# sxontheway/milliEye

Hardware: AMD Instinct MI355X
Metric: frames/sec YOLOv3-416+fusion @batch32, 1/2/4/8 MI355X; mAP@0.5 vs ref (higher is better)
Workload: dtype f32; 1 GPU; yolov3.cfg 416x416 fp32 inference, batch=32 per GPU, full milliEye: Darknet.forward -> NMS -> Network.forward mode 0 (R-CNN head + radar fusion, 2 radar boxes/frame) -> output rows, synthetic frames U[0,1), deterministic trained-like weights; stage=full, batch_per_gpu=32, global_batch=32, img_size=416, parallelism=frames sharded over 1 GPU(s), one process per GPU, no data-path collective, rccl_ranks=0, full=False, output_rows_last_step=6449, rois_last_step=6449

## Files before the change

### millieye_amd/csrc/conv.hip

```cpp
#include <stdlib.h>

#include "common.h"
#include "dma.h"

#include "conv32_common.h"

namespace me32 {
int launch_p8_tile(const ConvP& p, int tile, hipStream_t stream);
bool ws1x1_f32_eligible(const ConvP& p);
int launch_ws1x1_f32(const ConvP& p, hipStream_t stream);
bool ws3x3_f32_eligible(const ConvP& p);
int launch_ws3x3_f32(const ConvP& p, hipStream_t stream);
bool stem_mfma_eligible(const ConvP& p);
int launch_stem_mfma(const ConvP& p, hipStream_t stream);
}

namespace {

template <int BM, int BN, int BK, int WR, int WC, int ABL = 0, int PRIO = 0>
__global__ __launch_bounds__(256) void conv_igemm_f32(ConvP p) {
  static_assert(WR * WC == 4, "4 waves per workgroup");
  constexpr int TM = BM / WR, TN = BN / WC;
  constexpr int MT = TM / 32, NT = TN / 32;
  static_assert(MT >= 1 && NT >= 1, "wave tile must hold at least one 32x32 MFMA tile");
  constexpr int LP = BK + 4;
  constexpr int CH = BK / 4;
  constexpr int A_IT = (BM * CH + 255) / 256;
  constexpr int B_IT = (BN * CH + 255) / 256;

  extern __shared__ __attribute__((aligned(16))) float smem[];
  float* As = smem;
  float* Bs = smem + 2 * BM * LP;

  const int tid = threadIdx.x;
  const int lane = tid & 63;
  const int wave = tid >> 6;
  const int wr = wave / WC, wc = wave % WC;
// ... 1303 lines not shown
  p.cs = p.stages = p.tiles_m = p.tiles_n = p.bulk = p.gn = p.kord = 0;
  p.partial = nullptr;
  p.splitk = 1;
  p.sps = 0;
  p.counters = d->tile_counters_len > 0 ? d->tile_counters : nullptr;
  p.counters_len = p.counters ? d->tile_counters_len : 0;
  p.mask_cols = d->tap_mask_cols > 0 ? d->tap_mask_cols : 0;
  for (int i = 0; i < 4; ++i) p.tapmask[i] = d->tap_mask[i];
  return 0;
}

}

extern "C" {

int64_t me_conv2d_flops(const me_conv_desc* d) {
  if (!d) return 0;
  return 2ll * d->n * d->ho * d->wo * (int64_t)d->cout * d->ksize * d->ksize * d->cin;
}

int64_t me_conv2d_workspace_bytes(const me_conv_desc* d) {
  ConvP p;
  if (!d || fill_params(d, p) != 0 || d->cin <= 4) return 0;
  if ((d->tile >= 41 && d->tile <= 45) || d->tile == 47) {
    static const int shape[7][2] = {{128, 128}, {128, 64}, {64, 64}, {128, 32}, {256, 128}, {0, 0}, {64, 64}};
    const int bm = shape[d->tile - 41][0], bn = shape[d->tile - 41][1];
    const long long tiles = (long long)((p.M + bm - 1) / bm) * ((p.cout + bn - 1) / bn);
    const int split = d->split_k > 0 ? d->split_k : 4;
    return (int64_t)(tiles % 256) * split * bm * bn * (int64_t)sizeof(float);
  }
  const ConvPlan plan = plan_conv(p, d->tile, d->split_k > 0 ? d->split_k : kMaxSplit);
  const int split = d->split_k > 0 ? d->split_k : plan.splitk;
  return split > 1 ? (int64_t)split * p.M * p.cout * (int64_t)sizeof(float) : 0;
}

int me_conv2d_f32(const me_conv_desc* d, void* stream_) {
  hipStream_t stream = reinterpret_cast<hipStream_t>(stream_);
  ConvP p;
  int rc = fill_params(d, p);
  if (rc) return rc;
  ME_REQUIRE(d->x && d->wgt && d->scale && d->shift && d->y, ME_E_NULLPTR, "me_conv2d_f32: null tensor pointer");
  ME_REQUIRE(d->upsample == 1 || d->upsample == 2, ME_E_BADARG, "me_conv2d_f32: upsample must be 1 or 2");
  ME_REQUIRE(d->act >= 0 && d->act <= 2, ME_E_BADARG, "me_conv2d_f32: unknown activation %d", d->act);
  ME_REQUIRE(d->y_pitch >= d->cout, ME_E_BADARG, "me_conv2d_f32: y_pitch < cout");

  if (d->cin <= 4) {
    ME_REQUIRE(d->ksize == 3, ME_E_BADARG, "me_conv2d_f32: cin <= 4 needs ksize 3 (direct stem kernel)");
    ME_REQUIRE(d->cout <= SC_MAXCOUT, ME_E_TOOBIG, "me_conv2d_f32: small-cin kernel supports cout <= %d", SC_MAXCOUT);
    ME_REQUIRE(d->res == nullptr && d->upsample == 1, ME_E_BADARG,
               "me_conv2d_f32: small-cin kernel has no residual/upsample epilogue");
    ME_REQUIRE(d->x_nchw || d->x_pitch >= d->cin, ME_E_BADARG, "me_conv2d_f32: x_pitch < cin");
    ME_REQUIRE(me::aligned16(d->y), ME_E_ALIGN, "me_conv2d_f32: y not 16-byte aligned");
    if (d->tile == 0 && me32::stem_mfma_eligible(p)) return me32::launch_stem_mfma(p, stream);
    if (d->cin == 3 && (d->y_pitch & 3) == 0 && d->tile != 91) {
      const unsigned mb = (unsigned)((p.M + 255) / 256);
      if (d->cout % 32 == 0) {
        hipLaunchKernelGGL(conv_stem3_f32<32>, dim3(mb, d->cout / 32), dim3(256), 0, stream, p);
        return me::check_launch("conv_stem3_f32");
      }
      if (d->cout % 16 == 0) {
        hipLaunchKernelGGL(conv_stem3_f32<16>, dim3(mb, d->cout / 16), dim3(256), 0, stream, p);
        return me::check_launch("conv_stem3_f32");
      }
    }
    const long long threads = (long long)p.M * (((p.cout + 7) & ~7) >> 3);
    const unsigned blocks = (unsigned)((threads + 255) / 256);
    if (d->cin == 3)
// ... 101 lines not shown
```

### millieye_amd/engine.py

```python
import ctypes as C
import json
import os
import time

import torch

from . import hip, planner
from .planner import pick_tap_module

__all__ = ["DarknetEngine", "ConvWeights", "pick_tap_module", "invalidate_weights", "bump_versions"]

_EPOCH = [0]


def invalidate_weights():
    _EPOCH[0] += 1


def bump_versions(*tensors):
    torch.autograd.graph.increment_version(tensors)

_DTYPES = ("f32", "bf16", "f16")
_TORCH_HALF = {"bf16": torch.bfloat16, "f16": torch.float16}


class ConvWeights:

    def __init__(self, conv, bn=None, dtype="f32", cin_pad=0, cout_pad=0):
        self.conv, self.bn = conv, bn
        self.dtype, self.cin_pad, self.cout_pad = dtype, cin_pad, cout_pad
        self.wgt = self.scale = self.shift = None
        self.wgt_tiled = None
        self.want_rot = False
        self.rot = self.rot_tiled = None
        self.want_parity, self.parity, self.parity_stamp = False, None, None
        self._stamp = None

    def _sources(self):
        cp = self.conv._parameters
        ts = [cp["weight"]]
        if cp.get("bias") is not None:
            ts.append(cp["bias"])
        if self.bn is not None:
            bp, bb = self.bn._parameters, self.bn._buffers
            ts += [bp["weight"], bp["bias"], bb["running_mean"], bb["running_var"]]
        return ts

    def stamp(self):
        return tuple((t.data_ptr(), t._version) for t in self._sources()) + (_EPOCH[0],)

    def _prepare_packed_f32(self, device):
        conv, bn = self.conv, self.bn
        w = conv.weight
        cout, cin, k, k2 = w.shape
        if k != k2:
            return None
        srcs = [w] + [t for t in ((conv.bias,) if conv.bias is not None else ())]
        if bn is not None:
            srcs += [bn.weight, bn.bias, bn.running_mean, bn.running_var]
        if not all(t.device == device and t.dtype == torch.float32 and t.is_contiguous() for t in srcs):
            return None
        f32 = dict(device=device, dtype=torch.float32)
        realloc = self.wgt is None or self.wgt.device != device or tuple(self.wgt.shape) != (cout, k, k, cin) \
            or self.wgt.dtype != torch.float32
        if realloc:
            self.wgt = torch.empty((cout, k, k, cin), **f32)
            self.scale, self.shift = torch.empty(cout, **f32), torch.empty(cout, **f32)
            self.wgt_tiled = torch.empty((k * k, cin // 16, cout, 16), **f32) if cin % 16 == 0 else None
            self.rot = self.rot_tiled = None
        if self.want_rot and self.rot is None:
            self.rot = torch.empty((cin, k, k, cout), **f32)
            self.rot_tiled = torch.empty((k * k, cout // 16, cin, 16), **f32) if cout % 16 == 0 else None
        if realloc:
            self.parity = None
        if self.want_parity and k == 3 and self.parity is None:
            self.parity = torch.empty((4 * cin, 2, 2, cout), **f32)
        return "realloc" if realloc else True

    def _pack_desc(self, d):
        conv, bn = self.conv, self.bn
        ptr = lambda t: t.data_ptr() if t is not None else None
        cout, cin, k, _ = conv.weight.shape
        d.w, d.bias = conv.weight.data_ptr(), ptr(conv.bias)
        d.gamma, d.beta = ptr(bn.weight if bn is not None else None), ptr(bn.bias if bn is not None else None)
        d.mean, d.var = ptr(bn.running_mean if bn is not None else None), ptr(bn.running_var if bn is not None else None)
        d.ohwi, d.tiled = self.wgt.data_ptr(), ptr(self.wgt_tiled)
        d.rot, d.rot_tiled = ptr(self.rot if self.want_rot else None), ptr(self.rot_tiled if self.want_rot else None)
        d.scale, d.shift = self.scale.data_ptr(), self.shift.data_ptr()
        d.parity = ptr(self.parity if self.want_parity else None)
        d.cout, d.cin, d.ksize, d.eps = cout, cin, k, float(bn.eps) if bn is not None else 0.0
        return d

    def _refresh_packed_f32(self, device):
        done = self._prepare_packed_f32(device)
        if done is None:
            return None
        self.parity_stamp = None
        d = self._pack_desc(hip.PackDesc())
        hip.check(hip.lib().me_pack_conv_f32(d.w, d.cout, d.cin, d.ksize, d.bias, d.gamma, d.beta, d.mean, d.var, d.eps, d.ohwi,
                                             d.tiled, d.rot, d.rot_tiled, d.scale, d.shift, hip.stream_ptr()),
                  "me_pack_conv_f32")
        return done

    def refresh(self, device):
        stamp = self.stamp() + (self.want_rot,)
        if stamp == self._stamp and self.wgt is not None and self.wgt.device == device:
            return False
        dev = torch.device(device)
        if self.dtype == "f32" and not self.cin_pad and not self.cout_pad and dev.type == "cuda":
            if dev.index is None:
                dev = torch.device("cuda", torch.cuda.current_device())
            done = self._refresh_packed_f32(dev)
            if done is not None:
                self._stamp = stamp
                return done
        with torch.no_grad():
            w = self.conv.weight.detach().to(device=device, dtype=torch.float32)
            packed = w.permute(0, 2, 3, 1).contiguous()
            cout = w.shape[0]
            if self.bn is not None:
                g = self.bn.weight.detach().to(device, torch.float64)
                b = self.bn.bias.detach().to(device, torch.float64)
                mean = self.bn.running_mean.detach().to(device, torch.float64)
                var = self.bn.running_var.detach().to(device, torch.float64)
                scale = g / torch.sqrt(var + self.bn.eps)
                shift = b - mean * scale
                if self.conv.bias is not None:
# ... 112 lines not shown
            for cw, _ in stale:
                if cw.refresh(dev) == "realloc" and self._plans:
                    self._plans.clear()
            return
        if "realloc" in states and self._plans:
            self._plans.clear()
        descs = (hip.PackDesc * len(stale))()
        for d, (cw, _) in zip(descs, stale):
            cw._pack_desc(d)
        key = bytes(descs)
        cached = self.__dict__.get("_pack_table")
        if cached is None or cached[0] != key:
            total = int(hip.lib().me_pack_conv_plan(descs, len(stale)))
            if total <= 0:
                raise hip.MeError("me_pack_conv_plan: " + hip.lib().me_last_error().decode("utf-8", "replace"))
            table = torch.frombuffer(bytearray(bytes(descs)), dtype=torch.uint8).to(dev)
            cached = self._pack_table = (key, table, total, max(int(d.ksize) for d in descs))
        _, table, total, max_k = cached
        hip.check(hip.lib().me_pack_conv_batch_f32(table.data_ptr(), len(stale), total, max_k, hip.stream_ptr()),
                  "me_pack_conv_batch_f32")
        for cw, stamp in stale:
            cw._stamp = stamp
            cw.parity_stamp = stamp if cw.parity is not None else None

    def refresh_weights(self, device):
        fast = self.__dict__.get("_fast_sources")
        if fast is None:
            slots, bns = [], []
            for i, d in enumerate(self.model.module_defs):
                if d["type"] != "convolutional":
                    continue
                seq = self.model.module_list[i]
                conv = seq[0]
                slots.append((conv._parameters, "weight"))
                if conv._parameters.get("bias") is not None:
                    slots.append((conv._parameters, "bias"))
                if len(seq) > 1 and isinstance(seq[1], torch.nn.BatchNorm2d):
                    bn = seq[1]
                    bns.append(bn)
                    slots += [(bn._parameters, "weight"), (bn._parameters, "bias"), (bn._buffers, "running_mean"),
                              (bn._buffers, "running_var")]
            fast = self._fast_sources = (slots, bns)
            self._fast_stamp = None
        slots, bns = fast
        for bn in bns:
            if bn.training:
# ... 19 lines not shown
        return tuple([(t.data_ptr(), t._version) for t in [dct[key] for dct, key in fast[0]]]) + (str(device), _EPOCH[0])

    def _build(self, n, h, w, device, keep_raw=False):
        defs, tap = self.model.module_defs, self.tap_module
        half = self.dtype in _TORCH_HALF
        ops, tensors, out, yolo_rows = planner.lower(defs, int(self.model.hyperparams["channels"]), h, w, tap, half, keep_raw,
                                                     decode_last=os.environ.get("MILLIEYE_DECODE_LAST", "1") != "0")
        tap_tensor = out[tap] if tap is not None and tap < len(defs) else None
        total = planner.place(ops, tensors, n, tap_tensor, keep_raw)

        plan = _Plan()
        plan.n, plan.h, plan.w = n, h, w
        plan.arena = torch.empty(max(total, planner._ALIGN), dtype=torch.uint8, device=device)
        if plan.arena.data_ptr() % planner._ALIGN:
            raise RuntimeError("the caching allocator returned an arena that is not 256-byte aligned")
        plan.arena_bytes = total
        plan.dtype = self.dtype
        plan.rows = sum(yolo_rows)
        lib = hip.lib()
        self._emit(plan, ops, device, lib)
        self._attach_workspace(plan, device, lib)
        if _autotune_enabled():
            _autotune(plan, lib)
        plan.fused_blocks = []
        if half and _bneck_mode() != "0" and (_autotune_enabled() or _bneck_mode() == "force"):
            _fuse_bottlenecks(plan, ops, lib)
        if tap_tensor is not None:
            plan.tap = _typed_view(plan, tap_tensor, nchw=True)
            plan.tap_ptr, plan.tap_pitch = _view(plan, tap_tensor)
            plan.tap_shape = (tap_tensor.h, tap_tensor.w, tap_tensor.c)
        else:
            plan.tap = None
        return plan

    def _emit(self, plan, ops, device, lib):
        n, half = plan.n, plan.dtype in _TORCH_HALF
        half_type = hip.HALF_TYPES[_TORCH_HALF[plan.dtype]] if half else 0
        plan.num_classes = None
        plan.input_descs = []
        plan.yolo_raw = []
        plan.yolo_descs = []
        plan.conv_descs = []
        plan.conv_flops = 0
        plan.launches = launches = []
        for op in ops:
            kind, x, y, dsc = op["kind"], op.get("x"), op.get("y"), None
            if kind == "conv":
                op["launch"] = len(launches)
                dsc = op["desc"] = self._conv_desc(plan, op, device, half_type)
                fn = lib.me_conv2d_h16 if half else lib.me_conv2d_f32
            elif kind == "pool" and half:
                fn = lib.me_maxpool_h16
                args = (*_view(plan, x), *_view(plan, y), n, x.h, x.w, x.c, op["k"], op["s"],
                        0 if op["zero_ext"] else op["pad"], op["zero_ext"], op["ho"], op["wo"], half_type)
            elif kind == "pool":
                dsc = hip.PoolDesc()
                dsc.x, dsc.x_pitch = _view(plan, x)
                dsc.y, dsc.y_pitch = _view(plan, y)
                dsc.n, dsc.h, dsc.w, dsc.c = n, x.h, x.w, x.c
                dsc.size, dsc.stride, dsc.pad, dsc.zero_ext = op["k"], op["s"], (0 if op["zero_ext"] else op["pad"]), \
                    op["zero_ext"]
                dsc.ho, dsc.wo = op["ho"], op["wo"]
                fn = lib.me_maxpool_f32
            elif kind == "upsample":
                fn = lib.me_upsample_h16 if x.esize == 2 else lib.me_upsample_f32
# ... 23 lines not shown
            self._plans.clear()
        dsc = hip.Conv16Desc() if half else hip.ConvDesc()
        if x.external:
            dsc.x, dsc.x_pitch, dsc.x_nchw = None, x.c, 1
            plan.input_descs.append(dsc)
        else:
            dsc.x, dsc.x_pitch = _view(plan, x)
            dsc.x_nchw = 0
        dsc.wgt, dsc.scale, dsc.shift = cw.wgt.data_ptr(), cw.scale.data_ptr(), cw.shift.data_ptr()
        if op["res"] is not None:
            dsc.res, dsc.res_pitch = _view(plan, op["res"])
        else:
            dsc.res, dsc.res_pitch = None, 0
        dsc.y, dsc.y_pitch = _view(plan, y)
        dsc.n, dsc.h, dsc.w, dsc.cin = plan.n, x.h, x.w, x.c
        dsc.cout, dsc.ksize, dsc.stride, dsc.pad = cw.wgt.shape[0], op["k"], op["s"], op["pad"]
        dsc.ho, dsc.wo, dsc.act, dsc.upsample, dsc.tile = op["ho"], op["wo"], op["act"], op["ups"], 0
        dsc.split_k, dsc.workspace, dsc.workspace_bytes = 0, None, 0
        dsc.wgt_tiled = cw.wgt_tiled.data_ptr() if cw.wgt_tiled is not None else None
        if half:
            dsc.y_f32 = 1 if y.esize == 4 else 0
            dsc.half_type = half_type
        plan.conv_descs.append((op["module"], dsc))
        plan.conv_flops += 2 * plan.n * op["ho"] * op["wo"] * op["cout"] * op["k"] * op["k"] * (x.c - x.padded)
        return dsc

    def _yolo_desc(self, plan, op):
        x, i = op["x"], op["module"]
        yl = self.model.module_list[i][0]
        na, nc = yl.num_anchors, yl.num_classes
        if x.c != na * (nc + 5):
            raise ValueError(f"yolo {i}: {x.c} channels != {na}*({nc}+5)")
        dsc = hip.YoloDesc()
        dsc.x, dsc.x_pitch = _view(plan, x)
        dsc.out = None
        dsc.n, dsc.g, dsc.num_anchors, dsc.num_classes = plan.n, op["g"], na, nc
        dsc.rows_total, dsc.row_offset = plan.rows, op["row_offset"]
        stride = plan.h / op["g"]
        dsc.stride = stride
        for k, (aw, ah) in enumerate(yl.anchors):
            dsc.anchors[2 * k] = aw / stride
            dsc.anchors[2 * k + 1] = ah / stride
        plan.num_classes = nc
        plan.yolo_descs.append(dsc)
        plan.yolo_raw.append(_typed_view(plan, x, nchw=False))
        yl.img_dim = plan.h
# ... 201 lines not shown
    if _TUNE_FILE_LOADED[0]:
        return
    _TUNE_FILE_LOADED[0] = True
    try:
        with open(_tune_file()) as fh:
            for k, v in json.load(fh).items():
                _TUNE_CACHE[tuple(int(x) for x in k.split(","))] = (int(v[0]), int(v[1]))
    except (OSError, ValueError):
        pass


def _tune_save():
    path = _tune_file()
    try:
        os.makedirs(os.path.dirname(path), exist_ok=True)
        tmp = f"{path}.{os.getpid()}.tmp"
        with open(tmp, "w") as fh:
            json.dump({",".join(str(int(x)) for x in k): list(v) for k, v in _TUNE_CACHE.items()}, fh)
        os.replace(tmp, path)
    except OSError:
        pass


def _autotune(plan, lib):

    stream = hip.stream_ptr()
    _tune_load()
    bf16 = plan.dtype in _TORCH_HALF
    conv_fn = lib.me_conv2d_h16 if bf16 else lib.me_conv2d_f32
    todo, keyed = [], []
    for _m, d in plan.conv_descs:
        if d.cin <= 4:
            continue
        key = (d.n, d.h, d.w, d.cin, d.cout, d.ksize, d.stride, d.upsample, int(bool(d.res)))
        if bf16:
            key += (16 + d.y_f32 + 2 * d.half_type,)
        keyed.append((key, d))
        hit = _TUNE_CACHE.get(key)
        if hit is not None:
            d.tile, d.split_k = hit
        else:
            todo.append((key, d))

    def agree_on_rank0():
        import torch.distributed as dist
        if not (dist.is_available() and dist.is_initialized() and dist.get_world_size() > 1):
            return
        if os.environ.get("MILLIEYE_TUNE_SYNC", "0") not in ("1", "true", "on"):
            return
        box = [{k: (int(dd.tile), int(dd.split_k)) for k, dd in keyed} if dist.get_rank() == 0 else None]
        dist.broadcast_object_list(box, src=0)
        _TUNE_STATS["synced"] += 1
        for k, dd in keyed:
            hit0 = box[0].get(k)
            if hit0 is not None:
                dd.tile, dd.split_k = hit0
                _TUNE_CACHE[k] = hit0

    def ensure_workspace(nbytes):
        have = plan.conv_ws.numel() - 256 if plan.conv_ws is not None else 0
        if nbytes > have:
            plan.conv_ws = torch.empty(nbytes + 256, dtype=torch.uint8, device=plan.arena.device)
            have = nbytes
        ptr = plan.conv_ws.data_ptr() + (-plan.conv_ws.data_ptr()) % 256 if plan.conv_ws is not None else None
        for _m2, d2 in plan.conv_descs:
            if d2.cin > 4:
                d2.workspace, d2.workspace_bytes = ptr, have
        return have

    def scratch_of(d2):
        if not bf16 and d2.tile in _TUNE_TILES_TAIL + (47,):
            return int(lib.me_conv2d_workspace_bytes(C.byref(d2)))
        if bf16 and d2.tile >= 100:
            return int(lib.me_conv2d_h16_workspace_bytes(C.byref(d2)))
        return d2.split_k * d2.n * d2.ho * d2.wo * d2.cout * 4 if d2.split_k > 1 else 0

    def required():
        return max([scratch_of(d2) for _m2, d2 in plan.conv_descs if d2.cin > 4] + [0])

    _TUNE_STATS["measured"] += len(todo)
    if not todo:
        agree_on_rank0()
        ensure_workspace(required())
        return
    ws_bytes = plan.conv_ws.numel() - 256 if plan.conv_ws is not None else 0
    need = 0
    for _k, d in todo:
        slab = d.n * d.ho * d.wo * d.cout * 4
        if slab * 2 <= 512 * 2 ** 20:
            need = max(need, min(8 * slab, 512 * 2 ** 20))
        need = max(need, (128 if bf16 else 64) * 2 ** 20)
    ws_bytes = ensure_workspace(max(need, required()))

    def run(d, reps):
        for _ in range(reps):
            rc = conv_fn(C.byref(d), stream)
            if rc != 0:
                return False
        return True

    def timed(d, reps):
        a, b = torch.cuda.Event(enable_timing=True), torch.cuda.Event(enable_timing=True)
        a.record()
        ok = run(d, reps)
        b.record()
        torch.cuda.synchronize()
        return a.elapsed_time(b) / reps if ok else None

    t_end = time.perf_counter() + 0.3
    d0 = todo[0][1]
    d0.tile, d0.split_k = 0, 1
    while time.perf_counter() < t_end:
        run(d0, 5)
        torch.cuda.synchronize()
    for key, d in todo:
        hit = _TUNE_CACHE.get(key)
        if hit is not None:
            d.tile, d.split_k = hit
            continue
        slab = d.n * d.ho * d.wo * d.cout * 4
        stages = d.ksize * d.ksize * ((d.cin + 15) // 16)
        best = (float("inf"), 0, 1)
        cands = []
        tiles = _TUNE_TILES
        if bf16:
            stages = d.ksize * d.ksize * (d.cin // 32)
            tiles = _TUNE_TILES_BF16 if d.cin % 64 == 0 else _TUNE_TILES_BF16[:4] + (15,)
            if d.ksize == 3 and d.stride == 1 and d.upsample == 1 and d.wgt_tiled and not d.y_f32:
                tiles = tiles + _TUNE_TILES_P8
            no_ws = os.environ.get("MILLIEYE_NO_WS", "")
            if d.ksize == 1 and d.stride == 1 and d.upsample == 1 and not d.y_f32 and not d.res and "50" not in no_ws:
                tiles = tiles + (50,)
            if d.ksize == 3 and d.cin <= 64 and d.upsample == 1 and not d.y_f32 and "60" not in no_ws:
                tiles = tiles + (60,)
            if d.n * d.ho * d.wo <= _KW_MAX_POSITIONS and os.environ.get("MILLIEYE_NO_KW", "0") != "1":
                tiles = tiles + (40, 41)
        else:
            if d.cin % 16 == 0 and os.environ.get("MILLIEYE_TUNE_TAIL", "1") != "0":
                tiles = tiles + _TUNE_TILES_TAIL
            if d.ksize == 3 and d.stride == 1 and d.upsample == 1 and d.wgt_tiled:
                tiles = tiles + _TUNE_TILES_P8_F32
            no_ws32 = os.environ.get("MILLIEYE_NO_WS32", "")
            if d.ksize == 1 and d.stride == 1 and d.upsample == 1 and not d.res and d.act != hip.ACT_SIGMOID \
                    and d.cin in (64, 128, 256, 384, 512) and "50" not in no_ws32:
                tiles = tiles + (50,)
            if d.ksize == 3 and d.pad == 1 and d.cin in (32, 64) and d.upsample == 1 and d.act != hip.ACT_SIGMOID \
                    and "60" not in no_ws32:
                tiles = tiles + (60,)
        for tile in tiles:
            bm, bn = _TILE_SHAPES_BF16[tile] if (bf16 or tile >= 100 or tile in (50, 60)) else \
                {1: (128, 128), 2: (128, 64), 3: (64, 64), 4: (128, 32), 5: (256, 128), 7: (64, 64)}[tile % 40]
            ntiles = -(-d.n * d.ho * d.wo // bm) * -(-d.cout // bn)
            tail = not bf16 and tile in _TUNE_TILES_TAIL
            if tail and ntiles % 256 == 0:
                continue
            p8_split = False
            for split in (_TUNE_SPLITS[1:] if tail else (1,) if tile in (50, 60) or (bf16 and tile in (40, 41)) else _TUNE_SPLITS if tile < 100
                          else (1, 2, 3, 4) if p8_split else (1,)):
                d.tile, d.split_k = tile, split
                if tail or (tile >= 100 and split > 1):
                    if split > stages or scratch_of(d) > ws_bytes:
                        continue
                elif split > 1 and (split * slab > ws_bytes or ntiles * split > 4096 or split > stages):
                    continue
                if not run(d, 2):
                    continue
                ms = timed(d, 4)
                if ms is not None:
                    cands.append((ms, tile, split, split > 1 or tail))
        cands.sort()
        finalists = cands[:4]
        whole = [c for c in cands if not c[3]]
        if whole and whole[0] not in finalists:
            finalists.append(whole[0])
        score = {}
        for _round in range(3):
            for c in finalists:
                d.tile, d.split_k = c[1], c[2]
                ms = timed(d, 6)
                if ms is not None:
                    score.setdefault(c, []).append(ms)
        ranked = sorted((sorted(v)[len(v) // 2], c) for c, v in score.items())
        if os.environ.get("MILLIEYE_TUNE_VERBOSE"):
            import sys
            print("[tune]", key, " ".join(f"{c[1]}/{c[2]}:{1e3 * c[0]:.0f}>{1e3 * t:.0f}us" for t, c in ranked), file=sys.stderr, flush=True)
        if ranked:
            best = ranked[0]
            whole = [r for r in ranked if not r[1][3]]
            if best[1][3] and whole and best[0] > 0.98 * whole[0][0]:
                best = whole[0]
            best = (best[0], best[1][1], best[1][2])
        d.tile, d.split_k = best[1], best[2]
        _TUNE_CACHE[key] = (best[1], best[2])
    agree_on_rank0()
    ensure_workspace(required())
    _tune_save()


def _bneck_mode():
    return os.environ.get("MILLIEYE_BNECK", "1")


_BNECK_CACHE = {}
_BNECK_STATS = {"fused": 0, "kept": 0}


def _fuse_bottlenecks(plan, ops, lib):
    stream = hip.stream_ptr()
    launches = plan.launches
    conv_ops = [op for op in ops if op["kind"] == "conv"]
    index = {id(op): k for k, op in enumerate(ops)}
    pairs = []
    for a, b in zip(conv_ops, conv_ops[1:]):
        da, db = a["desc"], b["desc"]
        if not (index[id(b)] == index[id(a)] + 1 and b["x"] is a["y"]):
# ... 78 lines not shown
```

### millieye_amd/hip.py

```python
import ctypes as C
import os

import torch

__all__ = ["lib", "available", "default_device", "MeError"]

_HERE = os.path.dirname(os.path.abspath(__file__))
LIB_PATH = os.environ.get("MILLIEYE_HIP_LIB") or os.path.join(_HERE, "libmillieye_hip.so")

ACT_LINEAR, ACT_LEAKY, ACT_SIGMOID = 0, 1, 2


class MeError(RuntimeError):
    pass


class ConvDesc(C.Structure):
    _fields_ = [
        ("x", C.c_void_p), ("wgt", C.c_void_p), ("scale", C.c_void_p), ("shift", C.c_void_p),
        ("res", C.c_void_p), ("y", C.c_void_p),
        ("x_pitch", C.c_int64), ("res_pitch", C.c_int64), ("y_pitch", C.c_int64),
        ("n", C.c_int32), ("h", C.c_int32), ("w", C.c_int32), ("cin", C.c_int32),
        ("cout", C.c_int32), ("ksize", C.c_int32), ("stride", C.c_int32), ("pad", C.c_int32),
        ("ho", C.c_int32), ("wo", C.c_int32),
# ... 498 lines not shown
                continue
            if ms < best[0]:
                best = (ms, tile, split, masked)
        hit = _CONV_AUTO[key] = (best[1], best[2], best[3])
        _conv_auto_save()
    masked = len(hit) > 2 and hit[2]
    try:
        return conv2d(x_nhwc, wgt_packed, scale, shift, ksize, stride, pad, act, residual=residual, out=out, tile=hit[0],
                      split_k=hit[1], wgt_tiled=wgt_tiled, tap_masks=tap_masks if masked else None)
    except MeError:
        if hit[0] == 0 and not masked:
            raise
        _CONV_AUTO[key] = (0, 0, 0)
        return conv2d(x_nhwc, wgt_packed, scale, shift, ksize, stride, pad, act, residual=residual, out=out, wgt_tiled=wgt_tiled)


def tile_weights_f32(wgt_packed):
    cout, kh, kw, cin = wgt_packed.shape
    if cin % 16:
        raise MeError("tile_weights_f32: cin must be a multiple of 16")
    return wgt_packed.reshape(cout, kh * kw, cin // 16, 16).permute(1, 2, 0, 3).contiguous()


def tile_weights_h16(wgt_packed):
    cout, kh, kw, cin = wgt_packed.shape
    if cin % 32:
        raise MeError("tile_weights_h16: cin must be a multiple of 32")
    return wgt_packed.reshape(cout, kh * kw, cin // 32, 32).permute(1, 2, 0, 3).contiguous()


def conv2d_h16(x, wgt_packed, scale, shift, ksize, stride, pad, act, residual=None, upsample=1, out=None,
                x_nchw=False, y_f32=False, tile=0, split_k=0, half=torch.bfloat16, wgt_tiled=None, debug_ws=None, tap_masks=None):
    if not (isinstance(x, torch.Tensor) and x.is_cuda):
        raise MeError("x must be a CUDA tensor")
    if x_nchw:
        n, cin, h, w = x.shape
    else:
        n, h, w, cin = x.shape
    if cin > 4:
        half = x.dtype
    if half not in HALF_TYPES:
        raise MeError(f"me_conv2d_h16: 16-bit type must be bfloat16 or float16 (got {half})")
    want = torch.float32 if cin <= 4 else half
    if x.dtype != want or wgt_packed.dtype != want:
        raise MeError(f"me_conv2d_h16: x / wgt must be {want} for cin={cin} (got {x.dtype} / {wgt_packed.dtype})")
    cout = wgt_packed.shape[0]
# ... 411 lines not shown
```

Measured before the change: 1882 frames/s.

## Add Winograd F(2,3) fp32 conv path for stride-1 3x3 layers via autotune

Adds a 1-D Winograd F(2,3) convolution along the width axis for 3x3 stride-1 layers. A separate input-transform kernel writes the transformed activations to a workspace, and an MFMA GEMM kernel reads them with 12 taps per 16-channel chunk, keeps four accumulator sets and applies the inverse transform in the epilogue. Weights are transformed on the host in float64. The autotuner gains tiles 70/71 as candidates for eligible layers with cin>=64, which cuts MAC count by a quarter at the cost of an extra pass over the activations, a larger workspace and slightly different fp32 rounding.

```diff
diff --git a/millieye_amd/csrc/conv.hip b/millieye_amd/csrc/conv.hip
--- a/millieye_amd/csrc/conv.hip
+++ b/millieye_amd/csrc/conv.hip
@@ -13,6 +13,8 @@
 int launch_ws3x3_f32(const ConvP& p, hipStream_t stream);
 bool stem_mfma_eligible(const ConvP& p);
 int launch_stem_mfma(const ConvP& p, hipStream_t stream);
+int64_t wino_workspace_bytes(const me_conv_desc* d);
+int launch_wino_f32(const me_conv_desc* d, int store_mode, hipStream_t stream);
 }
 
 namespace {
@@ -1362,6 +1364,7 @@
 int64_t me_conv2d_workspace_bytes(const me_conv_desc* d) {
   ConvP p;
   if (!d || fill_params(d, p) != 0 || d->cin <= 4) return 0;
+  if (d->tile == 70 || d->tile == 71) return me32::wino_workspace_bytes(d);
   if ((d->tile >= 41 && d->tile <= 45) || d->tile == 47) {
     static const int shape[7][2] = {{128, 128}, {128, 64}, {64, 64}, {128, 32}, {256, 128}, {0, 0}, {64, 64}};
     const int bm = shape[d->tile - 41][0], bn = shape[d->tile - 41][1];
@@ -1383,6 +1386,8 @@
   ME_REQUIRE(d->upsample == 1 || d->upsample == 2, ME_E_BADARG, "me_conv2d_f32: upsample must be 1 or 2");
   ME_REQUIRE(d->act >= 0 && d->act <= 2, ME_E_BADARG, "me_conv2d_f32: unknown activation %d", d->act);
   ME_REQUIRE(d->y_pitch >= d->cout, ME_E_BADARG, "me_conv2d_f32: y_pitch < cout");
+
+  if (d->tile == 70 || d->tile == 71) return me32::launch_wino_f32(d, p.store_mode, stream);
 
   if (d->cin <= 4) {
     ME_REQUIRE(d->ksize == 3, ME_E_BADARG, "me_conv2d_f32: cin <= 4 needs ksize 3 (direct stem kernel)");
diff --git a/millieye_amd/csrc/conv_wino_f32.hip b/millieye_amd/csrc/conv_wino_f32.hip
--- /dev/null
+++ b/millieye_amd/csrc/conv_wino_f32.hip
@@ -0,0 +1,370 @@
+#include <hip/hip_runtime.h>
+#include <stdint.h>
+
+#include <type_traits>
+
+#include "common.h"
+#include "conv32_common.h"
+#include "dma.h"
+
+namespace {
+
+using namespace me_dma;
+
+struct WinoP {
+  const float* x;
+  float* v;
+  const float* pack;
+  const float* scale;
+  const float* shift;
+  const float* res;
+  float* y;
+  long long x_pitch, res_pitch, y_pitch;
+  int n, h, w, pairs, cin, cout, act;
+  int M;
+  int cs;
+  int tiles_m, tiles_n, gn;
+  unsigned hp_m, hp_s, p_m, p_s;
+  int store_mode;
+};
+
+__device__ __forceinline__ unsigned udiv_magic32(unsigned n, unsigned m, unsigned s) { return (__umulhi(n, m) + n) >> s; }
+
+void magic_u32(unsigned d, unsigned* m, unsigned* s) {
+  unsigned sh = 0;
+  while ((1ull << sh) < d) ++sh;
+  *s = sh;
+  *m = (unsigned)(((1ull << 32) * ((1ull << sh) - d)) / d + 1);
+}
+
+template <int N, class F, int I = 0>
+__device__ __forceinline__ void static_for(F&& f) {
+  if constexpr (I < N) {
+    f(std::integral_constant<int, I>{});
+    static_for<N, F, I + 1>(static_cast<F&&>(f));
+  }
+}
+
+__global__ __launch_bounds__(256) void wino_input_transform_f32(WinoP p) {
+  const int c4s = p.cin >> 2;
+  const long long total = (long long)p.M * c4s;
+  const long long idx = (long long)blockIdx.x * 256 + threadIdx.x;
+  if (idx >= total) return;
+  const int m = (int)(idx / c4s);
+  const int c = (int)(idx - (long long)m * c4s) * 4;
+  const int q = (int)udiv_magic32((unsigned)m, p.p_m, p.p_s);
+  const int pair = m - q * p.pairs;
+  const int col0 = 2 * pair - 1;
+  const float* xrow = p.x + (long long)q * p.w * p.x_pitch + c;
+  float4 d[4];
+#pragma unroll
+  for (int j = 0; j < 4; ++j) {
+    const int col = col0 + j;
+    d[j] = (unsigned)col < (unsigned)p.w ? *reinterpret_cast<const float4*>(xrow + (long long)col * p.x_pitch)
+                                         : make_float4(0.f, 0.f, 0.f, 0.f);
+  }
+  float* vp = p.v + (long long)m * 4 * p.cin + c;
+  *reinterpret_cast<float4*>(vp) = make_float4(d[0].x - d[2].x, d[0].y - d[2].y, d[0].z - d[2].z, d[0].w - d[2].w);
+  *reinterpret_cast<float4*>(vp + p.cin) = make_float4(d[1].x + d[2].x, d[1].y + d[2].y, d[1].z + d[2].z, d[1].w + d[2].w);
+  *reinterpret_cast<float4*>(vp + 2 * p.cin) = make_float4(d[2].x - d[1].x, d[2].y - d[1].y, d[2].z - d[1].z, d[2].w - d[1].w);
+  *reinterpret_cast<float4*>(vp + 3 * p.cin) = make_float4(d[1].x - d[3].x, d[1].y - d[3].y, d[1].z - d[3].z, d[1].w - d[3].w);
+}
+
+template <int BM, int BN, int WR, int WC>
+__global__ __launch_bounds__(64 * WR * WC, 1) void conv_wino_gemm_f32(WinoP p) {
+  constexpr int NW = WR * WC;
+  static_assert(NW == 4, "4 waves per workgroup");
+  constexpr int BK = 16, NST = 3, DEPTH = NST - 1, TAPS = 12;
+  constexpr int TM = BM / WR, TN = BN / WC;
+  constexpr int MT = TM / 32, NT = TN / 32;
+  constexpr int GA = BM / 16, G = (BM + BN) / 16;
+  constexpr int LPW = (G + NW - 1) / NW;
+  constexpr int LA = GA / NW;
+  constexpr int STAGE_F = LPW * NW * 256;
+  static_assert(GA % NW == 0, "A groups must split evenly over the waves");
+
+  extern __shared__ __attribute__((aligned(16))) float smem[];
+  const unsigned lds_base = (unsigned)(unsigned long long)(__attribute__((address_space(3))) float*)smem;
+
+  const int tid = threadIdx.x;
+  const int lane = tid & 63;
+  const int wave = __builtin_amdgcn_readfirstlane(tid >> 6);
+  const int wr = wave / WC, wc = wave % WC;
+  const int r32 = lane & 31, hh = lane >> 5;
+
+  int tile_m, tile_n;
+  {
+    const int nwg = p.tiles_m * p.tiles_n;
+    const int bid = blockIdx.x;
+    const int q = nwg >> 3, r = nwg & 7;
+    const int xcd = bid & 7, idx = bid >> 3;
+    const int wg = (xcd < r ? xcd * (q + 1) : r * (q + 1) + (xcd - r) * q) + idx;
+    const int per_panel = p.tiles_m * p.gn;
+    const int panel = wg / per_panel;
+    const int rr = wg - panel * per_panel;
+    const int left = p.tiles_n - panel * p.gn;
+    const int width = left < p.gn ? left : p.gn;
+    tile_m = rr / width;
+    tile_n = panel * p.gn + (rr - tile_m * width);
+    tile_m = __builtin_amdgcn_readfirstlane(tile_m);
+    tile_n = __builtin_amdgcn_readfirstlane(tile_n);
+  }
+  const int m0 = tile_m * BM, n0 = tile_n * BN;
+  const int hp = p.h * p.pairs;
+  const unsigned c4 = (unsigned)p.cin * 4u;
+  const long long row_elems = (long long)p.pairs * 4 * p.cin;
+
+  const int img0 = (int)udiv_magic32((unsigned)m0, p.hp_m, p.hp_s);
+  const long long img_elems = (long long)p.h * row_elems;
+  const u32x4 rsrc_a = make_rsrc(p.v + (long long)img0 * img_elems - row_elems);
+  const u32x4 rsrc_b = make_rsrc(p.pack + (long long)n0 * 16);
+  const unsigned b_step = (unsigned)p.cout * 64u;
+
+  const int lrow = lane >> 2;
+  unsigned v_row[3][LA];
+  unsigned v_b[LPW - LA];
+#pragma unroll
+  for (int j = 0; j < LPW; ++j) {
+    const int g = wave + NW * j;
+    const int row = g * 16 + lrow;
+    const int q = (lane & 3) ^ ((row >> 2) & 3);
+    if (j < LA) {
+      const int m = m0 + row;
+      unsigned base = kOobOffset;
+      bool ok[3] = {false, false, false};
+      if (m < p.M) {
+        const int nimg = (int)udiv_magic32((unsigned)m, p.hp_m, p.hp_s);
+        const int rem = m - nimg * hp;
+        const int oy = (int)udiv_magic32((unsigned)rem, p.p_m, p.p_s), pair = rem - oy * p.pairs;
+        const long long e = (long long)(nimg - img0) * img_elems + (long long)oy * row_elems + (long long)pair * 4 * p.cin;
+        base = (unsigned)(e * 4) + 16u * q;
+        ok[0] = oy >= 1;
+        ok[1] = true;
+        ok[2] = oy + 1 < p.h;
+      }
+#pragma unroll
+      for (int kr = 0; kr < 3; ++kr) v_row[kr][j < LA ? j : 0] = ok[kr] ? base : kOobOffset;
+    } else {
+      unsigned base = kOobOffset;
+      if (g < G) {
+        const int co_local = row - BM;
+        if (n0 + co_local < p.cout) base = (unsigned)co_local * 64u + 16u * q;
+      }
+      v_b[j >= LA ? j - LA : 0] = base;
+    }
+  }
+
+  f32x16 acc[4][MT][NT];
+#pragma unroll
+  for (int s = 0; s < 4; ++s)
+#pragma unroll
+    for (int i = 0; i < MT; ++i)
+#pragma unroll
+      for (int j = 0; j < NT; ++j)
+#pragma unroll
+        for (int e = 0; e < 16; ++e) acc[s][i][j][e] = 0.f;
+
+  constexpr unsigned STAGE_B = STAGE_F * 4u;
+  const unsigned wave_lds = __builtin_amdgcn_readfirstlane(lds_base + (unsigned)wave * 1024u);
+  const int sw = (r32 >> 2) & 3;
+  const int off0 = ((0 + hh) ^ sw) * 4, off1 = ((2 + hh) ^ sw) * 4;
+  const float* a_frag = smem + (wr * TM + r32) * BK;
+  const float* b_frag = smem + (BM + wc * TN + r32) * BK;
+
+  auto compute_stage = [&](auto set_c, const float* Ab, const float* Bb) {
+    constexpr int SET = decltype(set_c)::value;
+    float4 af[2][MT], bf[2][NT];
+#pragma unroll
+    for (int half = 0; half < 2; ++half) {
+      const int off = half ? off1 : off0;
+#pragma unroll
+      for (int i = 0; i < MT; ++i) af[half][i] = *reinterpret_cast<const float4*>(Ab + i * 32 * BK + off);
+#pragma unroll
+      for (int j = 0; j < NT; ++j) bf[half][j] = *reinterpret_cast<const float4*>(Bb + j * 32 * BK + off);
+    }
+    __builtin_amdgcn_sched_barrier(0);
+#pragma unroll
+    for (int half = 0; half < 2; ++half) {
+#pragma unroll
+      for (int kk = 0; kk < 4; ++kk)
+#pragma unroll
+        for (int i = 0; i < MT; ++i)
+#pragma unroll
+          for (int j = 0; j < NT; ++j) {
+            const float4 av = af[half][i], bv = bf[half][j];
+            const float a = kk == 0 ? av.x : kk == 1 ? av.y : kk == 2 ? av.z : av.w;
+            const float b = kk == 0 ? bv.x : kk == 1 ? bv.y : kk == 2 ? bv.z : bv.w;
+            acc[SET][i][j] = __builtin_amdgcn_mfma_f32_32x32x2f32(a, b, acc[SET][i][j], 0, 0, 0);
+          }
+    }
+  };
+
+  unsigned a_tap[TAPS], b_tap[TAPS];
+#pragma unroll
+  for (int t = 0; t < TAPS; ++t) {
+    a_tap[t] = (unsigned)(t / 4) * (unsigned)(row_elems * 4) + (unsigned)(t % 4) * c4;
+    b_tap[t] = (unsigned)t * (unsigned)p.cs * b_step;
+  }
+  unsigned ca = 0, cb = 0;
+  auto issue = [&](auto tap_c, unsigned ca_, unsigned cb_, unsigned lds_dst) {
+    constexpr int T = decltype(tap_c)::value;
+    unsigned v[LPW];
+#pragma unroll
+    for (int j = 0; j < LPW; ++j) v[j] = j < LA ? v_row[T / 4][j < LA ? j : 0] : v_b[j >= LA ? j - LA : 0];
+    dma_stage<LPW, LA, NW * 1024>(v, rsrc_a, rsrc_b, __builtin_amdgcn_readfirstlane(a_tap[T] + ca_),
+                                  __builtin_amdgcn_readfirstlane(b_tap[T] + cb_), lds_dst);
+  };
+  auto step = [&](auto tap_c, auto last_c) {
+    constexpr int T = decltype(tap_c)::value;
+    constexpr bool LAST = decltype(last_c)::value;
+    constexpr int SLOT = T % NST;
+    constexpr int YOUNGER = (LAST && TAPS - 1 - T < DEPTH - 1) ? TAPS - 1 - T : DEPTH - 1;
+    asm volatile("s_waitcnt vmcnt(%0) lgkmcnt(0)" ::"n"(LPW * YOUNGER) : "memory");
+    __builtin_amdgcn_s_barrier();
+    asm volatile("" ::: "memory");
+    constexpr unsigned DST = ((SLOT + DEPTH) % NST) * STAGE_B;
+    if constexpr (T + DEPTH < TAPS)
+      issue(std::integral_constant<int, (T + DEPTH) % TAPS>{}, ca, cb, wave_lds + DST);
+    else if constexpr (!LAST)
+      issue(std::integral_constant<int, (T + DEPTH) % TAPS>{}, ca + BK * 4u, cb + b_step, wave_lds + DST);
+    compute_stage(std::integral_constant<int, T % 4>{}, a_frag + SLOT * STAGE_F, b_frag + SLOT * STAGE_F);
+  };
+  auto chunk = [&](auto last_c) { static_for<TAPS>([&](auto tap_c) { step(tap_c, last_c); }); };
+  static_for<DEPTH>([&](auto tap_c) { issue(tap_c, ca, cb, wave_lds + decltype(tap_c)::value * STAGE_B); });
+  for (int c = 0; c + 1 < p.cs; ++c) {
+    chunk(std::false_type{});
+    ca += BK * 4u;
+    cb += b_step;
+  }
+  chunk(std::true_type{});
+
+  if (m0 + BM <= p.M && n0 + BN <= p.cout && (p.w & 1) == 0 && p.act != ME_ACT_SIGMOID) {
+    const float slope = p.act == ME_ACT_LEAKY ? 0.1f : 1.0f;
+    const long long ystep = p.y_pitch, rstep = p.res_pitch;
+#pragma unroll
+    for (int j = 0; j < NT; ++j) {
+      const int co = n0 + wc * TN + j * 32 + r32;
+      const float sc = p.scale[co], sh = p.shift[co];
+#pragma unroll
+      for (int i = 0; i < MT; ++i) {
+        const long long pix0 = 2ll * (m0 + wr * TM + i * 32 + 4 * hh);
+        float* yp = p.y + pix0 * ystep + co;
+        const float* rp = p.res ? p.res + pix0 * rstep + co : nullptr;
+#pragma unroll
+        for (int e = 0; e < 16; ++e) {
+          const float a0 = acc[0][i][j][e], a1 = acc[1][i][j][e], a2 = acc[2][i][j][e], a3 = acc[3][i][j][e];
+          const float t0 = ((a0 + a1) + a2) * sc + sh, t1 = ((a1 - a2) - a3) * sc + sh;
+          float o0 = fmaxf(t0, t0 * slope), o1 = fmaxf(t1, t1 * slope);
+          if (rp) {
+            o0 += rp[0];
+            o1 += rp[rstep];
+            rp += (e & 3) == 3 ? 10 * rstep : 2 * rstep;
+          }
+          me::store4(yp, o0, p.store_mode);
+          me::store4(yp + ystep, o1, p.store_mode);
+          yp += (e & 3) == 3 ? 10 * ystep : 2 * ystep;
+        }
+      }
+    }
+    return;
+  }
+#pragma unroll
+  for (int j = 0; j < NT; ++j) {
+    const int co = n0 + wc * TN + j * 32 + r32;
+    const bool co_ok = co < p.cout;
+    const float sc = co_ok ? p.scale[co] : 0.f;
+    const float sh = co_ok ? p.shift[co] : 0.f;
+#pragma unroll
+    for (int i = 0; i < MT; ++i) {
+#pragma unroll
+      for (int e = 0; e < 16; ++e) {
+        const int row = (e & 3) + 8 * (e >> 2) + 4 * hh;
+        const int m = m0 + wr * TM + i * 32 + row;
+        if (!co_ok || m >= p.M) continue;
+        const float a0 = acc[0][i][j][e], a1 = acc[1][i][j][e], a2 = acc[2][i][j][e], a3 = acc[3][i][j][e];
+        const int q = (int)udiv_magic32((unsigned)m, p.p_m, p.p_s);
+        const int pair = m - q * p.pairs;
+        const long long pix = (long long)q * p.w + 2 * pair;
+        float v0 = apply_act(((a0 + a1) + a2) * sc + sh, p.act);
+        if (p.res) v0 += p.res[pix * p.res_pitch + co];
+        p.y[pix * p.y_pitch + co] = v0;
+        if (2 * pair + 1 < p.w) {
+          float v1 = apply_act(((a1 - a2) - a3) * sc + sh, p.act);
+          if (p.res) v1 += p.res[(pix + 1) * p.res_pitch + co];
+          p.y[(pix + 1) * p.y_pitch + co] = v1;
+        }
+      }
+    }
+  }
+}
+
+template <int BM, int BN, int WR, int WC>
+int launch_gemm(WinoP& p, hipStream_t stream) {
+  constexpr int NW = WR * WC;
+  constexpr int LPW = ((BM + BN) / 16 + NW - 1) / NW;
+  const size_t lds = (size_t)3 * LPW * NW * 256 * sizeof(float);
+  p.tiles_m = (p.M + BM - 1) / BM;
+  p.tiles_n = (p.cout + BN - 1) / BN;
+  const long long panel_bytes = 1300ll * 1024, col_bytes = (long long)BN * 12 * p.cin * 4;
+  p.gn = p.tiles_n;
+  if (col_bytes * p.tiles_n > panel_bytes) {
+    const long long fit = panel_bytes / col_bytes;
+    p.gn = fit < 1 ? 1 : fit > p.tiles_n ? p.tiles_n : (int)fit;
+  }
+  const long long row_bytes = (long long)p.pairs * 4 * p.cin * 4;
+  const long long span_imgs = (BM - 1) / ((long long)p.h * p.pairs) + 2;
+  const long long a_max = span_imgs * p.h * row_bytes + 4 * row_bytes + 4ll * p.cin * 4;
+  const long long b_max = 12ll * p.cin * p.cout * 4 + 256ll * 64;
+  ME_REQUIRE(a_max < (1ll << 31) && b_max < (1ll << 31), ME_E_TOOBIG, "me_conv2d_f32: Winograd tile: offsets beyond 2^31");
+  const long long blocks = (long long)p.tiles_m * p.tiles_n;
+  ME_REQUIRE(blocks < (1ll << 31), ME_E_TOOBIG, "me_conv2d_f32: grid too large");
+  const long long tthreads = (long long)p.M * (p.cin / 4);
+  const long long tblocks = (tthreads + 255) / 256;
+  ME_REQUIRE(tblocks < (1ll << 31), ME_E_TOOBIG, "me_conv2d_f32: grid too large");
+  hipLaunchKernelGGL(wino_input_transform_f32, dim3((unsigned)tblocks), dim3(256), 0, stream, p);
+  int rc = me::check_launch("wino_input_transform_f32");
+  if (rc) return rc;
+  hipLaunchKernelGGL((conv_wino_gemm_f32<BM, BN, WR, WC>), dim3((unsigned)blocks), dim3(64 * NW), lds, stream, p);
+  return me::check_launch("conv_wino_gemm_f32");
+}
+
+}
+
+namespace me32 {
+
+int64_t wino_workspace_bytes(const me_conv_desc* d) {
+  if (!d || d->ksize != 3 || d->stride != 1 || d->pad != 1 || d->cin % 16 != 0 || d->n <= 0 || d->h <= 0 || d->w <= 0) return 0;
+  return (int64_t)d->n * d->h * ((d->w + 1) / 2) * 4 * d->cin * (int64_t)sizeof(float);
+}
+
+int launch_wino_f32(const me_conv_desc* d, int store_mode, hipStream_t stream) {
+  ME_REQUIRE(d->ksize == 3 && d->stride == 1 && d->pad == 1 && d->upsample == 1 && !d->x_nchw, ME_E_BADARG,
+             "me_conv2d_f32: tile %d (Winograd F(2,3)) needs ksize 3, stride 1, pad 1, upsample 1, NHWC input", d->tile);
+  ME_REQUIRE(d->cin % 16 == 0, ME_E_BADARG, "me_conv2d_f32: tile %d needs cin %% 16 == 0 (cin=%d)", d->tile, d->cin);
+  ME_REQUIRE(d->split_k <= 1 && d->tap_mask_cols <= 0, ME_E_BADARG, "me_conv2d_f32: tile %d has no K split and no tap masks", d->tile);
+  ME_REQUIRE(d->x_pitch >= d->cin && d->x_pitch % 4 == 0, ME_E_ALIGN, "me_conv2d_f32: x_pitch must be >= cin, %% 4");
+  ME_REQUIRE(!d->res || d->res_pitch >= d->cout, ME_E_BADARG, "me_conv2d_f32: res_pitch < cout");
+  ME_REQUIRE(d->wgt_tiled != nullptr, ME_E_NULLPTR, "me_conv2d_f32: tile %d reads the Winograd pack from wgt_tiled", d->tile);
+  const int64_t need = wino_workspace_bytes(d);
+  ME_REQUIRE(d->workspace != nullptr, ME_E_NULLPTR, "me_conv2d_f32: tile %d needs a workspace of %lld bytes", d->tile, (long long)need);
+  ME_REQUIRE(d->workspace_bytes >= need, ME_E_BADARG, "me_conv2d_f32: tile %d needs a workspace of %lld bytes", d->tile,
+             (long long)need);
+  ME_REQUIRE(me::aligned16(d->x) && me::aligned16(d->wgt_tiled) && me::aligned16(d->workspace), ME_E_ALIGN,
+             "me_conv2d_f32: x / wgt_tiled / workspace not 16-byte aligned");
+  WinoP p;
+  p.x = d->x; p.v = reinterpret_cast<float*>(d->workspace); p.pack = d->wgt_tiled;
+  p.scale = d->scale; p.shift = d->shift; p.res = d->res; p.y = d->y;
+  p.x_pitch = d->x_pitch; p.res_pitch = d->res_pitch; p.y_pitch = d->y_pitch;
+  p.n = d->n; p.h = d->h; p.w = d->w; p.pairs = (d->w + 1) / 2; p.cin = d->cin; p.cout = d->cout; p.act = d->act;
+  const long long rows = (long long)d->n * d->h * p.pairs;
+  ME_REQUIRE(rows < (1ll << 31), ME_E_TOOBIG, "me_conv2d_f32: too many output pixels");
+  p.M = (int)rows;
+  p.cs = d->cin / 16;
+  magic_u32((unsigned)(p.h * p.pairs), &p.hp_m, &p.hp_s);
+  magic_u32((unsigned)p.pairs, &p.p_m, &p.p_s);
+  p.tiles_m = p.tiles_n = p.gn = 0;
+  p.store_mode = store_mode;
+  return d->tile == 70 ? launch_gemm<64, 64, 2, 2>(p, stream) : launch_gemm<128, 32, 4, 1>(p, stream);
+}
+
+}
diff --git a/millieye_amd/engine.py b/millieye_amd/engine.py
--- a/millieye_amd/engine.py
+++ b/millieye_amd/engine.py
@@ -34,6 +34,7 @@
         self.want_rot = False
         self.rot = self.rot_tiled = None
         self.want_parity, self.parity, self.parity_stamp = False, None, None
+        self.wino = None
         self._stamp = None
 
     def _sources(self):
@@ -67,7 +68,7 @@
             self.wgt = torch.empty((cout, k, k, cin), **f32)
             self.scale, self.shift = torch.empty(cout, **f32), torch.empty(cout, **f32)
             self.wgt_tiled = torch.empty((k * k, cin // 16, cout, 16), **f32) if cin % 16 == 0 else None
-            self.rot = self.rot_tiled = None
+            self.rot = self.rot_tiled = self.wino = None
         if self.want_rot and self.rot is None:
             self.rot = torch.empty((cin, k, k, cout), **f32)
             self.rot_tiled = torch.empty((k * k, cout // 16, cin, 16), **f32) if cout % 16 == 0 else None
@@ -102,7 +103,21 @@
                   "me_pack_conv_f32")
         return done
 
+    def wino_pack(self):
+        if self.wino is None:
+            self.wino = hip.wino_weights_f32(self.wgt)
+        return self.wino
+
     def refresh(self, device):
+        done = self._refresh_packed(device)
+        if done and self.wino is not None:
+            if done == "realloc" or self.wino.device != self.wgt.device:
+                self.wino = None
+            else:
+                self.wino.copy_(hip.wino_weights_f32(self.wgt))
+        return done
+
+    def _refresh_packed(self, device):
         stamp = self.stamp() + (self.want_rot,)
         if stamp == self._stamp and self.wgt is not None and self.wgt.device == device:
             return False
@@ -261,6 +276,8 @@
         for cw, stamp in stale:
             cw._stamp = stamp
             cw.parity_stamp = stamp if cw.parity is not None else None
+            if cw.wino is not None:
+                cw.wino.copy_(hip.wino_weights_f32(cw.wgt))
 
     def refresh_weights(self, device):
         fast = self.__dict__.get("_fast_sources")
@@ -326,6 +343,12 @@
         self._attach_workspace(plan, device, lib)
         if _autotune_enabled():
             _autotune(plan, lib)
+        if not half and _wino_mode() == "force":
+            _force_wino(plan, lib)
+        used = {m for p in list(self._plans.values()) + [plan] for m, d in p.conv_descs if d.tile in hip.WINO_TILES}
+        for m, cw in self._weights.items():
+            if m not in used:
+                cw.wino = None
         plan.fused_blocks = []
         if half and _bneck_mode() != "0" and (_autotune_enabled() or _bneck_mode() == "force"):
             _fuse_bottlenecks(plan, ops, lib)
@@ -345,6 +368,7 @@
         plan.yolo_raw = []
         plan.yolo_descs = []
         plan.conv_descs = []
+        plan.conv_cw = {}
         plan.conv_flops = 0
         plan.launches = launches = []
         for op in ops:
@@ -414,6 +438,7 @@
             dsc.y_f32 = 1 if y.esize == 4 else 0
             dsc.half_type = half_type
         plan.conv_descs.append((op["module"], dsc))
+        plan.conv_cw[op["module"]] = cw
         plan.conv_flops += 2 * plan.n * op["ho"] * op["wo"] * op["cout"] * op["k"] * op["k"] * (x.c - x.padded)
         return dsc
 
@@ -661,12 +686,56 @@
         pass
 
 
+def _wino_mode():
+    return os.environ.get("MILLIEYE_WINO", "1")
+
+
+def _wino_eligible(d):
+    return d.ksize == 3 and d.stride == 1 and d.pad == 1 and d.upsample == 1 and not d.x_nchw and d.cin % 16 == 0 \
+        and d.tap_mask_cols <= 0
+
+
+def _sync_pack(plan, module, d):
+    cw = plan.conv_cw[module]
+    pack = cw.wino_pack() if d.tile in hip.WINO_TILES else cw.wgt_tiled
+    d.wgt_tiled = pack.data_ptr() if pack is not None else None
+
+
+def _ensure_workspace(plan, nbytes):
+    have = plan.conv_ws.numel() - 256 if plan.conv_ws is not None else 0
+    if nbytes > have:
+        plan.conv_ws = torch.empty(nbytes + 256, dtype=torch.uint8, device=plan.arena.device)
+        have = nbytes
+    ptr = plan.conv_ws.data_ptr() + (-plan.conv_ws.data_ptr()) % 256 if plan.conv_ws is not None else None
+    for _m2, d2 in plan.conv_descs:
+        if d2.cin > 4:
+            d2.workspace, d2.workspace_bytes = ptr, have
+    return have
+
+
+def _force_wino(plan, lib):
+    need = plan.conv_ws.numel() - 256 if plan.conv_ws is not None else 0
+    for m, d in plan.conv_descs:
+        if _wino_eligible(d):
+            d.tile, d.split_k = hip.WINO_TILES[0], 1
+            _sync_pack(plan, m, d)
+            need = max(need, int(lib.me_conv2d_workspace_bytes(C.byref(d))))
+    _ensure_workspace(plan, need)
+
+
 def _autotune(plan, lib):
 
     stream = hip.stream_ptr()
     _tune_load()
     bf16 = plan.dtype in _TORCH_HALF
     conv_fn = lib.me_conv2d_h16 if bf16 else lib.me_conv2d_f32
+    wino = not bf16 and _wino_mode() == "1"
+    module_of = {C.addressof(d): m for m, d in plan.conv_descs}
+
+    def sync_pack(d):
+        if not bf16:
+            _sync_pack(plan, module_of[C.addressof(d)], d)
+
     todo, keyed = [], []
     for _m, d in plan.conv_descs:
         if d.cin <= 4:
@@ -676,8 +745,11 @@
             key += (16 + d.y_f32 + 2 * d.half_type,)
         keyed.append((key, d))
         hit = _TUNE_CACHE.get(key)
+        if hit is not None and not bf16 and hit[0] in hip.WINO_TILES and not (wino and _wino_eligible(d)):
+            hit = None
         if hit is not None:
             d.tile, d.split_k = hit
+            sync_pack(d)
         else:
             todo.append((key, d))
 
@@ -694,21 +766,14 @@
             hit0 = box[0].get(k)
             if hit0 is not None:
                 dd.tile, dd.split_k = hit0
+                sync_pack(dd)
                 _TUNE_CACHE[k] = hit0
 
     def ensure_workspace(nbytes):
-        have = plan.conv_ws.numel() - 256 if plan.conv_ws is not None else 0
-        if nbytes > have:
-            plan.conv_ws = torch.empty(nbytes + 256, dtype=torch.uint8, device=plan.arena.device)
-            have = nbytes
-        ptr = plan.conv_ws.data_ptr() + (-plan.conv_ws.data_ptr()) % 256 if plan.conv_ws is not None else None
-        for _m2, d2 in plan.conv_descs:
-            if d2.cin > 4:
-                d2.workspace, d2.workspace_bytes = ptr, have
-        return have
+        return _ensure_workspace(plan, nbytes)
 
     def scratch_of(d2):
-        if not bf16 and d2.tile in _TUNE_TILES_TAIL + (47,):
+        if not bf16 and d2.tile in _TUNE_TILES_TAIL + (47,) + hip.WINO_TILES:
             return int(lib.me_conv2d_workspace_bytes(C.byref(d2)))
         if bf16 and d2.tile >= 100:
             return int(lib.me_conv2d_h16_workspace_bytes(C.byref(d2)))
@@ -729,6 +794,10 @@
         if slab * 2 <= 512 * 2 ** 20:
             need = max(need, min(8 * slab, 512 * 2 ** 20))
         need = max(need, (128 if bf16 else 64) * 2 ** 20)
+        if wino and _wino_eligible(d) and d.cin >= 64:
+            v_bytes = d.n * d.h * ((d.w + 1) // 2) * 4 * d.cin * 4
+            if v_bytes <= 512 * 2 ** 20:
+                need = max(need, v_bytes)
     ws_bytes = ensure_workspace(max(need, required()))
 
     def run(d, reps):
@@ -749,6 +818,7 @@
     t_end = time.perf_counter() + 0.3
     d0 = todo[0][1]
     d0.tile, d0.split_k = 0, 1
+    sync_pack(d0)
     while time.perf_counter() < t_end:
         run(d0, 5)
         torch.cuda.synchronize()
@@ -756,6 +826,7 @@
         hit = _TUNE_CACHE.get(key)
         if hit is not None:
             d.tile, d.split_k = hit
+            sync_pack(d)
             continue
         slab = d.n * d.ho * d.wo * d.cout * 4
         stages = d.ksize * d.ksize * ((d.cin + 15) // 16)
@@ -779,6 +850,8 @@
                 tiles = tiles + _TUNE_TILES_TAIL
             if d.ksize == 3 and d.stride == 1 and d.upsample == 1 and d.wgt_tiled:
                 tiles = tiles + _TUNE_TILES_P8_F32
+            if wino and _wino_eligible(d) and d.cin >= 64:
+                tiles = tiles + hip.WINO_TILES
             no_ws32 = os.environ.get("MILLIEYE_NO_WS32", "")
             if d.ksize == 1 and d.stride == 1 and d.upsample == 1 and not d.res and d.act != hip.ACT_SIGMOID \
                     and d.cin in (64, 128, 256, 384, 512) and "50" not in no_ws32:
@@ -788,16 +861,19 @@
                 tiles = tiles + (60,)
         for tile in tiles:
             bm, bn = _TILE_SHAPES_BF16[tile] if (bf16 or tile >= 100 or tile in (50, 60)) else \
+                {70: (64, 64), 71: (128, 32)}[tile] if tile in hip.WINO_TILES else \
                 {1: (128, 128), 2: (128, 64), 3: (64, 64), 4: (128, 32), 5: (256, 128), 7: (64, 64)}[tile % 40]
+            wino_tile = not bf16 and tile in hip.WINO_TILES
             ntiles = -(-d.n * d.ho * d.wo // bm) * -(-d.cout // bn)
             tail = not bf16 and tile in _TUNE_TILES_TAIL
             if tail and ntiles % 256 == 0:
                 continue
             p8_split = False
-            for split in (_TUNE_SPLITS[1:] if tail else (1,) if tile in (50, 60) or (bf16 and tile in (40, 41)) else _TUNE_SPLITS if tile < 100
-                          else (1, 2, 3, 4) if p8_split else (1,)):
+            for split in (_TUNE_SPLITS[1:] if tail else (1,) if tile in (50, 60) or wino_tile or (bf16 and tile in (40, 41))
+                          else _TUNE_SPLITS if tile < 100 else (1, 2, 3, 4) if p8_split else (1,)):
                 d.tile, d.split_k = tile, split
-                if tail or (tile >= 100 and split > 1):
+                sync_pack(d)
+                if tail or wino_tile or (tile >= 100 and split > 1):
                     if split > stages or scratch_of(d) > ws_bytes:
                         continue
                 elif split > 1 and (split * slab > ws_bytes or ntiles * split > 4096 or split > stages):
@@ -816,6 +892,7 @@
         for _round in range(3):
             for c in finalists:
                 d.tile, d.split_k = c[1], c[2]
+                sync_pack(d)
                 ms = timed(d, 6)
                 if ms is not None:
                     score.setdefault(c, []).append(ms)
@@ -830,6 +907,7 @@
                 best = whole[0]
             best = (best[0], best[1][1], best[1][2])
         d.tile, d.split_k = best[1], best[2]
+        sync_pack(d)
         _TUNE_CACHE[key] = (best[1], best[2])
     agree_on_rank0()
     ensure_workspace(required())
diff --git a/millieye_amd/hip.py b/millieye_amd/hip.py
--- a/millieye_amd/hip.py
+++ b/millieye_amd/hip.py
@@ -544,6 +544,19 @@
     return wgt_packed.reshape(cout, kh * kw, cin // 16, 16).permute(1, 2, 0, 3).contiguous()
 
 
+WINO_TILES = (70, 71)
+
+
+def wino_weights_f32(wgt_packed):
+    cout, kh, kw, cin = wgt_packed.shape
+    if (kh, kw) != (3, 3) or cin % 16:
+        raise MeError("wino_weights_f32: 3x3 filters with cin a multiple of 16")
+    g = wgt_packed.to(torch.float64)
+    g0, g1, g2 = g[:, :, 0], g[:, :, 1], g[:, :, 2]
+    u = torch.stack((g0, (g0 + g1 + g2) / 2, (g0 - g1 + g2) / 2, g2), dim=2)
+    return u.to(torch.float32).reshape(cout, 12, cin // 16, 16).permute(1, 2, 0, 3).contiguous()
+
+
 def tile_weights_h16(wgt_packed):
     cout, kh, kw, cin = wgt_packed.shape
     if cin % 32:
```

Result: no change. 1882 frames/s (-0.0%).
